# ikmb/vcf2prot

Measured on AMD Instinct MI355X. Metric: amino-acids written/sec, higher is better.
Workload: dtype u8

## Files before the change

### vcf2prot_amd/csrc/stitch_device.hpp

```cpp
#pragma once
#include <hip/hip_runtime.h>
#include <stdint.h>
#include "stitch_kernels.h"

namespace v2p {

typedef uint32_t u32x4 __attribute__((ext_vector_type(4)));
struct __attribute__((packed, aligned(1))) unaligned16 { u32x4 v; };

__device__ __forceinline__ u32x4 gather16(uint64_t addr)
{
    typedef const __attribute__((address_space(1))) unaligned16* gptr;
    return reinterpret_cast<gptr>(addr)->v;
}

struct __attribute__((packed, aligned(4))) dwaligned16 { u32x4 v; };
__device__ __forceinline__ u32x4 gather16_dw(uint64_t addr)
{
    typedef const __attribute__((address_space(1))) dwaligned16* gptr;
    typedef const __attribute__((address_space(1))) uint32_t* dptr;
    const uint64_t base = addr & ~3ull;
    const uint32_t sh = uint32_t(addr) & 3u;
    const u32x4 v = reinterpret_cast<gptr>(base)->v;
    const uint32_t e = *reinterpret_cast<dptr>(base + 16u);
// ... 100 lines not shown
            const uint32_t b0 = payload[src], b1 = payload[src + len - 1u];
            asm volatile("" :: "v"(b0), "v"(b1));
        }
    };
#pragma unroll
    for (uint32_t k = 0; k < TOUCH_CHUNKS_PER_WAVE; ++k) payload_lines(d[k]);
    for (uint32_t k = 0; k < TOUCH_CHUNKS_PER_WAVE; ++k) {
        const uint64_t n = (ch[k].dst_n >> 48) & uint64_t(CHUNK_N_MASK);
        const uint64_t tb = ch[k].task_begin & TB_IDX_MASK;
        for (uint64_t i = tb + 64u + lane; i < tb + n && i < n_desc; i += 64u) payload_lines(desc[i]);
    }
#pragma unroll
    for (uint32_t k = 0; k < TOUCH_CHUNKS_PER_WAVE; ++k) asm volatile("" :: "v"(d[k]));
}

}
```

### vcf2prot_amd/csrc/stitch_kernels.h

```cpp
#pragma once
#include <hip/hip_runtime.h>
#include <stdint.h>
#include "sir_pack.hpp"

namespace v2p {

enum : uint32_t {
    STATUS_BAD_CODE = 1,
    STATUS_RES_OOB = 2,
    STATUS_SRC_OOB = 3,
    STATUS_NOT_CONTIGUOUS = 4
};
constexpr unsigned long long STATUS_CLEAN = ~0ull;
constexpr int STITCH_TASKS_PER_LANE = 4;
constexpr uint32_t DOTS_BYTES = 64u * 1024u + 128u;

struct StitchArgs {
    const uint64_t* desc;
    uint64_t        n_desc;
    const Chunk*    chunks;
    uint32_t        n_chunks;
    const uint8_t*  src0;
    uint64_t        src0_len;
    const uint8_t*  src1;
// ... 4 lines not shown
    const uint8_t*  dots;
    const Chunk*    next_chunks = nullptr;
    uint32_t        n_next = 0;
    uint32_t        store_sc1 = 0;
    uint64_t        opt_phase_bytes = 0;
    uint32_t        opt_phase_min_chunks = 0;
    int32_t         opt_store_sc1 = -1;
    uint32_t        opt_touch = 0;
    uint32_t        rows = 0;
    uint64_t        img_desc = 0, img_bytes = 0;
    hipStream_t     aux_stream = nullptr;
    hipEvent_t      ev_fork = nullptr, ev_join = nullptr;
    uint32_t        opt_dual = 0;
    uint64_t*       stage = nullptr;
    uint32_t        stage_chunks = 0;
    const uint64_t* stage_cur = nullptr;
    uint64_t*       stage_next = nullptr;
    uint32_t        phase_chunks = 0;
};

uint32_t stitch_stage_chunks(const StitchArgs& args, int nontemporal);

struct OrderedArgs {
    const uint8_t*  code;
    const uint64_t* start_pos;
    const uint64_t* length;
    const uint64_t* start_pos_res;
    uint64_t        n_tasks;
    const uint8_t*  ref;
    const uint8_t*  alt;
    uint8_t*        res;
    uint64_t        esize;
};

struct ValidateArgs {
    const uint8_t*  code;
// ... 30 lines not shown
```

### vcf2prot_amd/csrc/stitch_kernels.hip

```cpp
#include <hip/hip_runtime.h>
#include <utility>
#include <vector>
#include <stdint.h>
#include <stdlib.h>
#include <mutex>
#include "stitch_kernels.h"
#include "stitch_device.hpp"

namespace v2p {

__device__ __forceinline__ u32x4 overwrite_tail(u32x4 v, u32x4 ld, uint32_t ja, bool take)
{
    const uint64_t x = ~0ull << (8u * (ja & 7u));
    const uint64_t mlo = (take && ja < 8u) ? x : 0ull;
    const uint64_t mhi = take ? (ja < 8u ? ~0ull : x) : 0ull;
    const uint32_t k0 = uint32_t(mlo), k1 = uint32_t(mlo >> 32), k2 = uint32_t(mhi), k3 = uint32_t(mhi >> 32);
    v[0] = (v[0] & ~k0) | (ld[0] & k0);
    v[1] = (v[1] & ~k1) | (ld[1] & k1);
    v[2] = (v[2] & ~k2) | (ld[2] & k2);
    v[3] = (v[3] & ~k3) | (ld[3] & k3);
    return v;
}

template <bool DW>
// ... 1009 lines not shown
    std::lock_guard<std::mutex> lk(mu);
    if (!bufs[dev]) {
        uint8_t* p = nullptr;
        *err = hipMalloc(reinterpret_cast<void**>(&p), DOTS_BYTES);
        if (*err != hipSuccess) return nullptr;
        *err = hipMemset(p, '.', DOTS_BYTES);
        if (*err == hipSuccess) *err = hipDeviceSynchronize();
        if (*err != hipSuccess) { (void)hipFree(p); return nullptr; }
        bufs[dev] = p;
    }
    return bufs[dev];
}


__global__ __launch_bounds__(256) void touch_image_kernel(const uint64_t* __restrict__ desc, const Chunk* __restrict__ chunks, uint32_t n_chunks, uint64_t n_desc,
                                                          const uint8_t* __restrict__ payload, uint64_t payload_len, uint64_t* __restrict__ stage)
{
    touch_chunks(desc, chunks, touch_wave_first(blockIdx.x & 7u, (blockIdx.x >> 3) * 4u + (threadIdx.x >> 6)), n_chunks, n_desc, payload, payload_len, threadIdx.x & 63u, stage);
}

static hipError_t launch_stitch_range(const StitchArgs& args, hipStream_t stream, int nontemporal, uint32_t max_blocks);

#ifdef V2P_BENCH_VARIANTS
__global__ void idle_kernel(uint32_t us)
{
    const uint64_t t0 = __builtin_readcyclecounter();
    while (__builtin_readcyclecounter() - t0 < uint64_t(us) * 100u) __builtin_amdgcn_s_sleep(64);
}
#endif

static uint64_t phase_plan(const StitchArgs& a, int nontemporal, uint32_t max_blocks, bool staged, bool* ride_out)
{
    *ride_out = false;
// ... 13 lines not shown
    per = per < per_min ? per_min : (per & ~7ull);
    const bool no_touch = (a.opt_touch & 1u) != 0, own_touch = (a.opt_touch & 2u) != 0;
    *ride_out = !own_touch && !no_touch && (nontemporal & 4) != 0 && (nontemporal & 48) == 48 && !(nontemporal & 2);
    return per;
}

uint32_t stitch_stage_chunks(const StitchArgs& args, int nontemporal)
{
    bool ride = false;
    const uint64_t per = phase_plan(args, nontemporal, 0, true, &ride);
    const int wsel = (nontemporal >> 28) & 3;
    if (!ride || !(nontemporal & 8) || wsel != 0 || (args.opt_touch & 4u) != 0 || args.opt_dual || per == 0 || per > 0x7FFFFFFFull) return 0;
    return uint32_t(per < args.n_chunks ? per : ((uint64_t(args.n_chunks) + 7u) & ~7ull));
}

hipError_t launch_stitch(const StitchArgs& args, hipStream_t stream, int nontemporal, uint32_t max_blocks)
{
    if (args.n_chunks == 0) return hipSuccess;
    StitchArgs a = args;
    hipError_t err = hipSuccess;
    a.dots = device_dots(&err);
    if (!a.dots) return err;
    a.rows = (nontemporal & 8) != 0;
    const uint64_t img_desc = a.img_desc ? a.img_desc : a.n_desc, img_bytes = a.img_bytes ? a.img_bytes : a.out_len;
    const bool rich = image_is_rich(img_desc, img_bytes);
    a.store_sc1 = a.opt_store_sc1 >= 0 ? uint32_t(a.opt_store_sc1 != 0) : uint32_t(!rich);
    bool ride = false;
    const uint64_t per = phase_plan(a, nontemporal, max_blocks, args.stage != nullptr && a.rows, &ride);
    if (per == 0) return launch_stitch_range(a, stream, nontemporal, max_blocks);
    const bool no_touch = (a.opt_touch & 1u) != 0;
    const int wsel = (nontemporal >> 28) & 3;
    if (ride && wsel == 0 && (a.opt_touch & 4u) != 0 && per <= 0x7FFFFFFFull) {
        const uint32_t n0 = uint32_t(args.n_chunks < per ? args.n_chunks : per);
        hipLaunchKernelGGL(touch_image_kernel, dim3(8u * ((touch_waves_per_xcd(n0) + 3u) / 4u)), dim3(256), 0, stream, a.desc, a.chunks, n0, a.n_desc, a.src1, a.src1_len, nullptr);
        a.phase_chunks = uint32_t(per);
        return launch_stitch_range(a, stream, nontemporal, 0);
    }
    if (ride && wsel == 0 && a.opt_dual && a.aux_stream && a.ev_fork && a.ev_join && args.n_chunks >= 4u * per) {
        const uint64_t half = (per / 2u) & ~7ull;
        std::vector<std::pair<uint64_t, uint32_t>> pieces;
        for (uint64_t c0 = 0; c0 < args.n_chunks; ) {
            uint64_t nc = pieces.size() == 1u ? (half / 2u) & ~7ull : half;
            if (nc == 0u) nc = 8u;
            if (nc > args.n_chunks - c0) nc = args.n_chunks - c0;
            pieces.emplace_back(c0, uint32_t(nc));
            c0 += nc;
        }
        err = hipEventRecord(a.ev_fork, stream);
        if (err == hipSuccess) err = hipStreamWaitEvent(a.aux_stream, a.ev_fork, 0);
        if (err != hipSuccess) return err;
        for (size_t i = 0; i < pieces.size(); ++i) {
            hipStream_t s = (i & 1u) ? a.aux_stream : stream;
            a.chunks = args.chunks + pieces[i].first;
            a.n_chunks = pieces[i].second;
            a.next_chunks = nullptr; a.n_next = 0;
            if (i + 2u < pieces.size()) { a.next_chunks = args.chunks + pieces[i + 2u].first; a.n_next = pieces[i + 2u].second; }
            if (i < 2u) hipLaunchKernelGGL(touch_image_kernel, dim3(8u * ((touch_waves_per_xcd(a.n_chunks) + 3u) / 4u)), dim3(256), 0, s, a.desc, a.chunks, a.n_chunks, a.n_desc, a.src1, a.src1_len, nullptr);
            err = launch_stitch_range(a, s, nontemporal, 0);
            if (err != hipSuccess) return err;
        }
        err = hipEventRecord(a.ev_join, a.aux_stream);
        if (err == hipSuccess) err = hipStreamWaitEvent(stream, a.ev_join, 0);
        return err != hipSuccess ? err : hipGetLastError();
    }
    const bool staged = ride && a.rows && wsel == 0 && args.stage != nullptr && per <= args.stage_chunks;
    uint32_t phase = 0;
    for (uint64_t c0 = 0; c0 < args.n_chunks; c0 += per, ++phase) {
        const uint32_t nc = uint32_t(args.n_chunks - c0 < per ? args.n_chunks - c0 : per);
        a.chunks = args.chunks + c0;
        a.n_chunks = nc;
        a.next_chunks = nullptr; a.n_next = 0;
        if (ride && c0 + per < args.n_chunks) {
            a.next_chunks = args.chunks + c0 + per;
            a.n_next = uint32_t(args.n_chunks - (c0 + per) < per ? args.n_chunks - (c0 + per) : per);
        }
        a.stage_cur = nullptr; a.stage_next = nullptr;
        if (staged) {
            a.stage_cur = args.stage + uint64_t(phase & 1u) * args.stage_chunks * STAGE_SLOTS;
            a.stage_next = args.stage + uint64_t((phase + 1u) & 1u) * args.stage_chunks * STAGE_SLOTS;
        }
        if (!no_touch && (!ride || c0 == 0)) hipLaunchKernelGGL(touch_image_kernel, dim3(8u * ((touch_waves_per_xcd(nc) + 3u) / 4u)), dim3(256), 0, stream, a.desc, a.chunks, nc, a.n_desc, a.src1, a.src1_len,
                                                                 staged ? const_cast<uint64_t*>(a.stage_cur) : nullptr);
        err = launch_stitch_range(a, stream, nontemporal, 0);
        if (err != hipSuccess) return err;
#ifdef V2P_BENCH_VARIANTS
        if (const char* e = getenv("V2P_PHASE_GAP_US")) hipLaunchKernelGGL(idle_kernel, dim3(1), dim3(64), 0, stream, uint32_t(atoi(e)));
        if (getenv("V2P_PHASE_SYNC")) (void)hipStreamSynchronize(stream);
#endif
    }
    return hipGetLastError();
}

static hipError_t launch_stitch_range(const StitchArgs& a, hipStream_t stream, int nontemporal, uint32_t max_blocks)
{
    hipError_t err = hipSuccess;
    const int nt = nontemporal & 1;
    const int var = (nontemporal >> 12) & 0xF;
// ... 124 lines not shown
```

### vcf2prot_amd/csrc/stitch_wave.hip

```cpp
#include <hip/hip_runtime.h>
#include <stdint.h>
#include <stdlib.h>
#include "stitch_kernels.h"
#include "stitch_device.hpp"

namespace v2p {

struct __attribute__((aligned(16))) WRec {
    uint32_t a_lo, a_hi;
    uint32_t se;
    uint32_t lit;
};
constexpr uint32_t WREC_NOLIT = 0xFFFFu;

__device__ __forceinline__ uint64_t wrec_adj(const WRec& t) { return (uint64_t(t.a_hi) << 32) | t.a_lo; }

__device__ __forceinline__ u32x4 put_byte(u32x4 v, uint32_t q, uint32_t byte)
{
    const uint32_t sh = 8u * (q & 3u), m = 0xFFu << sh, bv = byte << sh, k = q >> 2;
    v[0] = k == 0u ? (v[0] & ~m) | bv : v[0];
    v[1] = k == 1u ? (v[1] & ~m) | bv : v[1];
    v[2] = k == 2u ? (v[2] & ~m) | bv : v[2];
    v[3] = k == 3u ? (v[3] & ~m) | bv : v[3];
    return v;
// ... 33 lines not shown
    v[2] = (ld[2] & m[2]) | (v[2] & ~m[2]);
    v[3] = (ld[3] & m[3]) | (v[3] & ~m[3]);
    return v;
}

#ifndef V2P_WAVE_OCC
#define V2P_WAVE_OCC 8
#endif
template <int WPG, bool NT, bool SC1 = false, bool RIMG = false, bool STG = false>
__global__ __launch_bounds__(64 * WPG, V2P_WAVE_OCC) void stitchw_kernel(const uint64_t* __restrict__ p_desc, const Chunk* __restrict__ p_chunks,
                                                            const uint8_t* __restrict__ p_src0, const uint8_t* __restrict__ p_src1,
                                                            uint8_t* __restrict__ p_out, unsigned long long* __restrict__ p_status,
                                                            const uint8_t* __restrict__ p_dots,
                                                            uint32_t n_chunks, uint64_t n_desc, uint64_t src0_len, uint64_t src1_len, uint64_t out_len,
                                                            const Chunk* __restrict__ p_next, uint32_t n_next, uint32_t phase_chunks,
                                                            const uint64_t* __restrict__ p_stage = nullptr, uint64_t* __restrict__ p_stage_next = nullptr)
{
    static_assert(!STG || (RIMG && WPG == 1), "staged descriptors: rows images, one wave per workgroup");
    constexpr uint32_t ROWS = CHUNK_BYTES_WAVE / 1024u;
    static_assert(ROWS <= 16u, "a lane's map bytes and record indices are packed four rows to a register");
    constexpr uint32_t ND = (ROWS + 3u) / 4u;
    struct WaveLds {
        uint32_t map32[64u * ND];
        WRec rec[CHUNK_TASKS_WAVE + 4];
        u32x4 patch[CHUNK_TASKS_WAVE + 1];
    };
    __shared__ __attribute__((aligned(16))) WaveLds s_all[WPG];
    __shared__ u32x4 s_mask[17];
    __shared__ u32x4 s_one[17];

    const uint32_t lane = threadIdx.x & 63u;
// ... 1 lines not shown
    uint32_t c = blockIdx.x * uint32_t(WPG) + wid;
    if (WPG == 1 && phase_chunks != 0u) {
        const uint32_t tw = 8u * touch_waves_per_xcd(phase_chunks), per = tw + phase_chunks;
        const uint32_t g = blockIdx.x / per, r = blockIdx.x - g * per;
        if (r < tw) {
            const uint64_t base = uint64_t(g + 1u) * phase_chunks;
            if (base < n_chunks)
                touch_chunks(p_desc, p_chunks + base, touch_wave_first(r & 7u, r >> 3), uint32_t(n_chunks - base < phase_chunks ? n_chunks - base : phase_chunks),
                             n_desc, p_src1, src1_len, lane);
            return;
        }
        c = g * phase_chunks + (r - tw);
        if (c >= n_chunks) return;
    } else if (c >= n_chunks) {
        const uint32_t first_wg = (((n_chunks + uint32_t(WPG) - 1u) / uint32_t(WPG)) + 7u) & ~7u;
        if (blockIdx.x >= first_wg)
            touch_chunks(p_desc, p_next, touch_wave_first(blockIdx.x & 7u, ((blockIdx.x - first_wg) >> 3) * uint32_t(WPG) + wid), n_next, n_desc, p_src1, src1_len, lane,
                         STG ? p_stage_next : nullptr);
        return;
    }
    WaveLds& L = s_all[wid];
    uint64_t d_stg = 0ull;
    if (STG) d_stg = p_stage[uint64_t(c) * STAGE_SLOTS + lane];
    const uint64_t tb_raw = p_chunks[c].task_begin, dn = p_chunks[c].dst_n;
    if (!(dn & CHUNK_WAVE)) return;
    const uint64_t tb = RIMG ? tb_raw & TB_IDX_MASK : tb_raw;
    const uint32_t hskip = RIMG ? uint32_t(tb_raw >> TB_IDX_BITS) & PIECE_MAX : 0u;
    const uint32_t tclip = RIMG ? uint32_t(tb_raw >> (TB_IDX_BITS + TB_SKIP_BITS)) : 0u;
    const uint32_t n_hdr = uint32_t(dn >> 48) & CHUNK_N_MASK;
    if (RIMG != ((dn & CHUNK_CLIP) != 0ull)) { if (lane == 0u) report(p_status, tb, STATUS_RES_OOB); return; }
    const uint32_t n1 = RIMG ? uint32_t(dn & CHUNK_N1_MASK) : 0u;
    const uint64_t dst = RIMG ? dn & (DST_MASK & ~CHUNK_N1_MASK) : dn & DST_MASK;
    const uint32_t head = RIMG ? 0u : uint32_t(dst) & 15u;
// ... 217 lines not shown
    if (const char* e = getenv("V2P_WAVE_SUB")) sub = uint32_t(strtoul(e, nullptr, 10));
#endif
    if (sub == 0 || sub > a.n_chunks) sub = a.n_chunks;
    sub = (sub + 7u) & ~7u;
    for (uint32_t c0 = 0; c0 < a.n_chunks; c0 += sub) {
        const uint32_t nc = a.n_chunks - c0 < sub ? a.n_chunks - c0 : sub;
        const Chunk* ch = a.chunks + c0;
        const bool last = c0 + sub >= a.n_chunks;
        const uint32_t n_next = last && a.next_chunks ? a.n_next : 0u;
        const uint32_t tw = n_next ? touch_waves_per_xcd(n_next) : 0u;
#define V2P_LW(WW, NTT) hipLaunchKernelGGL((stitchw_kernel<WW, NTT>), dim3(tw ? ((((nc + (WW) - 1u) / (WW)) + 7u) & ~7u) + 8u * ((tw + (WW) - 1u) / (WW)) : (nc + (WW) - 1u) / (WW)), dim3(64 * (WW)), 0, stream, \
        a.desc, ch, a.src0, a.src1, a.out, a.status, a.dots, nc, a.n_desc, a.src0_len, a.src1_len, a.out_len, a.next_chunks, n_next, 0u)
#define V2P_LWR(NTT, SCC) hipLaunchKernelGGL((stitchw_kernel<1, NTT, SCC, true>), dim3(tw ? (((nc + 7u) & ~7u) + 8u * tw) : nc), dim3(64), 0, stream, \
        a.desc, ch, a.src0, a.src1, a.out, a.status, a.dots, nc, a.n_desc, a.src0_len, a.src1_len, a.out_len, a.next_chunks, n_next, 0u, nullptr, nullptr)
#define V2P_LWS(NTT, SCC) hipLaunchKernelGGL((stitchw_kernel<1, NTT, SCC, true, true>), dim3(tw ? (((nc + 7u) & ~7u) + 8u * tw) : nc), dim3(64), 0, stream, \
        a.desc, ch, a.src0, a.src1, a.out, a.status, a.dots, nc, a.n_desc, a.src0_len, a.src1_len, a.out_len, a.next_chunks, n_next, 0u, a.stage_cur, a.stage_next)
        if (a.rows && a.stage_cur && c0 == 0u && nc == a.n_chunks) {
            if (nt && a.store_sc1) V2P_LWS(true, true); else if (nt) V2P_LWS(true, false); else V2P_LWS(false, false);
        } else if (a.rows) { if (nt && a.store_sc1) V2P_LWR(true, true); else if (nt) V2P_LWR(true, false); else V2P_LWR(false, false); }
#ifdef V2P_BENCH_VARIANTS
        else if (waves_per_group == 4) { if (nt) V2P_LW(4, true); else V2P_LW(4, false); }
        else if (waves_per_group == 2) { if (nt) V2P_LW(2, true); else V2P_LW(2, false); }
#endif
        else if (nt && a.store_sc1) hipLaunchKernelGGL((stitchw_kernel<1, true, true>), dim3(tw ? (((nc + 7u) & ~7u) + 8u * tw) : nc), dim3(64), 0, stream,
                                                      a.desc, ch, a.src0, a.src1, a.out, a.status, a.dots, nc, a.n_desc, a.src0_len, a.src1_len, a.out_len, a.next_chunks, n_next, 0u);
        else { if (nt) V2P_LW(1, true); else V2P_LW(1, false); }
#undef V2P_LW
#undef V2P_LWR
#undef V2P_LWS
    }
    return hipGetLastError();
// ... 11 lines not shown
```

### vcf2prot_amd/csrc/v2p_api.hip

```cpp
#include <hip/hip_runtime.h>
#include <cstdint>
#include <cstdio>
#include <cstring>
#include <atomic>
#include <chrono>
#include <condition_variable>
#include <cstdlib>
#include <functional>
#include <memory>
#include <mutex>
#include <new>
#include <string>
#include <thread>
#include <vector>

#include "../../include/vcf2prot_hip.h"
#include "sir_pack.hpp"
#include "stitch_kernels.h"
#include "build_kernels.h"
#include "build_rows.h"
#include "dense_pieces.h"
#ifdef V2P_BENCH_VARIANTS
#include "patch_image.h"
#include "bench/v2p_bench.h"
// ... 139 lines not shown
    uint32_t tile_slots = 0;
    uint64_t tiles_n = 0;
    const uint32_t* tiles_count = nullptr;
    const uint64_t* tiles_res_base = nullptr;
    const uint8_t* payload_dev = nullptr;
    struct v2p_stream* from_stream = nullptr;
    bool orphaned = false;
    uint64_t pieces_src0_len = 0, pieces_src1_len = 0;
    DevBuf d_tiles, d_cover, d_pad, d_order;
    DevBuf d_pieces, d_chunks2;
    bool executed = false;
    uint64_t n_pieces = 0;
    int pieces_state = 0;
    PinnedBuf h_sum;
    DevBuf d_stage;
    bool pad_image = false;
    bool desc_swapped = false;
    uint64_t desc_slots = 0, pad_n_tiles = 0;
    uint32_t pad_K = 0;
    const uint64_t* pad_tdbase = nullptr;
    uint32_t n_slices = 0;
    uint64_t slice_chunk0[V2P_MAX_SLICES + 1] = {};
    uint64_t slice_desc[V2P_MAX_SLICES] = {}, slice_bytes[V2P_MAX_SLICES] = {};
    hipEvent_t ev_os[2 + 2 * V2P_MAX_SLICES] = {};
    hipEvent_t ev_aux[2] = {};
    hipEvent_t ev_par[V2P_MAX_SLICES] = {};
    bool os_ahead = false;
    float os_build_ms = 0.f;
    double os_wall_ms = 0.0;
    int os_kernel = 0;
// ... 1306 lines not shown
    } else if (n_chunks) HIP_TRY(c, hipMemcpyAsync(b->d_chunks.ptr(), a.chunks_tmp, n_chunks * sizeof(Chunk), hipMemcpyDeviceToDevice, c->stream), "D2D(chunks)");
    HIP_TRY(c, hipEventRecord(guard.ev[7], c->stream), "hipEventRecord");
    b->img.hap_out_begin.assign(n_h + 1, 0);
    HIP_TRY(c, hipMemcpyAsync(b->img.hap_out_begin.data(), b->d_hap.ptr(), (n_h + 1) * 8, hipMemcpyDeviceToHost, c->stream), "D2H(hap_begin)");
    rc = collect_status(c, b->d_status);
    if (rc) { (void)hipMemsetAsync(b->d_status.ptr(), 0xFF, 8, c->stream); return rc; }
    float ms0 = 0.f, ms1 = 0.f, ms2 = 0.f;
    (void)hipEventElapsedTime(&ms0, guard.ev[0], guard.ev[1]);
    (void)hipEventElapsedTime(&ms1, guard.ev[4], guard.ev[5]);
    (void)hipEventElapsedTime(&ms2, guard.ev[6], guard.ev[7]);
    if (build_ms) *build_ms = ms0 + ms_parse + ms1 + ms2;
    guard.ok = true;
    b->n_desc = n_desc; b->n_chunks = n_chunks; b->n_payload = v.n_alt; b->payload_dev = v.alt; b->out_bytes = out_bytes; b->n_haps = n_h;
    b->launch_hint = (mode == ROWS_DENSE ? 2 : 4) | 8 | 16 | 32 | (1 << 6) | (1 << 8);
    b->uses_proteome = true;
    b->finalized = true;
    b->n_slices = 0;
    return V2P_OK;
}

struct CheckErr { std::string msg; int64_t index = -1; int operator()(int code, const std::string& m, int64_t i = -1) { msg = m; index = i; return code; } };
static int check_stream_nolock(const v2p_ctx* c, const v2p_txstream* s, bool* fasta_out, std::vector<uint32_t>* arena_len, std::vector<uint64_t>* hap_out_begin, CheckErr& fail)
{
    if (!s->hap_tx_begin || (s->n_tx && (!s->tx_proteome_off || !s->tx_ref_len || !s->tx_res_len || !s->tx_task_begin || !s->tx_alt_begin)) ||
        (s->n_tasks && (!s->code || !s->start_pos || !s->length || !s->start_pos_res)) || (s->n_alt && !s->alt))
        return fail(V2P_ERR_INVALID_ARG, "null argument");
    if (s->hap_tx_begin[s->n_haps] != s->n_tx || (s->n_tx && (s->tx_task_begin[s->n_tx] != s->n_tasks || s->tx_alt_begin[s->n_tx] != s->n_alt)))
        return fail(V2P_ERR_INVALID_ARG, "stream offsets do not add up");
    if (s->hap_tx_begin[0] != 0) return fail(V2P_ERR_INVALID_ARG, "hap_tx_begin does not start at 0", 0);
    for (uint64_t h = 0; h < s->n_haps; ++h)
        if (s->hap_tx_begin[h + 1] < s->hap_tx_begin[h] || s->hap_tx_begin[h + 1] > s->n_tx)
// ... 207 lines not shown
    b->img.hap_out_begin.assign(n_h + 1, 0);
    HIP_TRY(c, hipMemcpyAsync(b->img.hap_out_begin.data(), b->d_hap.ptr(), (n_h + 1) * 8, hipMemcpyDeviceToHost, c->stream), "D2H(hap_begin)");
    rc = collect_status(c, b->d_status);
    float ms = 0.f, ms2 = 0.f;
    (void)hipEventElapsedTime(&ms, e0, e1);
    (void)hipEventElapsedTime(&ms2, e2, e3);
    ms += ms2;
    if (rc) { (void)hipMemsetAsync(b->d_status.ptr(), 0xFF, 8, c->stream); return rc; }
    guard.ok = true;
    if (build_ms) *build_ms = ms;
    b->n_desc = n_desc; b->n_chunks = n_chunks; b->n_payload = s->n_alt; b->payload_dev = b->d_payload.ptr(); b->out_bytes = out_bytes; b->n_haps = n_h;
    b->n_slices = 0;
    const int tpt = meta[3] <= 256u ? 1 : (meta[3] <= 512u ? 2 : 4);
    b->launch_hint = ((meta[0] & 2u) ? 2 : 0) | ((meta[0] & 4u) ? 4 : 0) | ((meta[0] & 1u) ? 0 : 16) | (meta[2] ? 0 : 32) | ((meta[1] ? 2 : 1) << 6) | (tpt << 8);
    b->uses_proteome = true;
    b->finalized = true;
    return V2P_OK;
#endif
}

#ifdef V2P_BENCH_VARIANTS
static int build_patch_image(v2p_batch* b, const DevStreamView& v, float* build_ms, bool own_stream_copy, uint64_t known_out_bytes)
{
    v2p_ctx* c = b->ctx;
    const uint64_t n_tx = v.n_tx, n_h = v.n_haps;
    struct Cleanup {
        hipEvent_t ev[2] = {nullptr, nullptr};
        DevBuf scratch;
        v2p_batch* b;
        bool ok = false, own;
        Cleanup(v2p_batch* b_, bool own_) : b(b_), own(own_) {}
// ... 75 lines not shown
    HIP_TRY(c, hipStreamSynchronize(c->stream), "hipStreamSynchronize");
    if (st != STATUS_CLEAN) {
        (void)hipMemsetAsync(b->d_status.ptr(), 0xFF, 8, c->stream);
        if (uint32_t(st & 0xFFu) == STATUS_PATCH_DECLINED) return c->fail(V2P_ERR_UNSUPPORTED, "a 8 KiB window of the result holds more segments or patches than a patch image's chunk (kernel 7 builds a dense image)", int64_t(st >> 8));
        const int code = reason_to_err(uint32_t(st & 0xFFu));
        return c->fail(code, std::string("device: ") + err_name(code) + " at descriptor " + std::to_string(st >> 8), int64_t(st >> 8));
    }
    float ms = 0.f;
    (void)hipEventElapsedTime(&ms, guard.ev[0], guard.ev[1]);
    if (build_ms) *build_ms = ms;
    guard.ok = true;
    b->n_desc = totals[0]; b->patch_segs = totals[0]; b->patch_patches = totals[1];
    b->n_chunks = n_chunks; b->n_payload = v.n_alt; b->payload_dev = v.alt; b->out_bytes = out_bytes; b->n_haps = n_h;
    b->launch_hint = 0; b->is_patch = true;
    b->uses_proteome = true;
    b->finalized = true;
    b->n_slices = 0;
    return V2P_OK;
}
#endif

struct v2p_stream {
    v2p_ctx* ctx = nullptr;
    DevBuf buf, alt;
    DevStreamView v;
    uint64_t out_bytes = 0;
    std::vector<uint64_t> hap_out_begin;
    DevBuf tiles;
    uint32_t tile_K = 0;
    uint64_t n_tiles = 0;
    const uint64_t* tile_res_base = nullptr;
// ... 126 lines not shown
    if (bpt >= double(WAVE_BYTES_PER_TASK)) return ROWS_WAVE;
    return ctx_variant(st->ctx) != 28u && tiles_possible(st) ? ROWS_TILES : ROWS_DENSE;
}

static int batch_reset_locked(v2p_batch* b, bool wait)
{
    v2p_ctx* c = b->ctx;
    HIP_TRY(c, hipSetDevice(c->device), "hipSetDevice");
    if (wait) HIP_TRY(c, hipStreamSynchronize(c->stream), "hipStreamSynchronize");
    b->img = ImageBuilder();
    b->finalized = false; b->uses_proteome = false; b->hap_open = false;
    b->n_desc = b->n_chunks = b->n_payload = b->out_bytes = b->n_haps = 0;
    b->payload_dev = nullptr; b->n_slices = 0; b->launch_hint = 0; b->is_patch = false; b->patch_segs = b->patch_patches = 0;
    b->is_tiles = false; b->tile_slots = 0; b->tiles_n = 0; b->tiles_count = nullptr; b->tiles_res_base = nullptr;
    b->pad_image = false; b->desc_slots = 0; b->pad_tdbase = nullptr; b->pieces_state = 0; b->executed = false;
    b->z_ready = false; b->z_begin.clear();
    b->os_kernel = 0; b->os_build_ms = 0.f; b->os_wall_ms = 0.0; b->os_ahead = false;
    stream_detach(b); b->orphaned = false;
    if (b->desc_swapped) { std::swap(b->d_desc, b->d_pad); b->desc_swapped = false; }
    return V2P_OK;
}

int v2p_batch_reset(v2p_batch* b)
{
    if (!b) return V2P_ERR_INVALID_ARG;
    std::lock_guard<std::mutex> lk(b->ctx->mu);
    const int rc = batch_reset_locked(b, true);
    b->d_z.release(); b->d_zws.release(); b->d_zbegin.release();
    return rc;
}
// ... 44 lines not shown

static void dual_of(v2p_ctx* c, StitchArgs& a)
{
    if (ctx_variant(c) != 19u) return;
    if (!c->exec_aux && hipStreamCreateWithFlags(&c->exec_aux, hipStreamNonBlocking) != hipSuccess) { c->exec_aux = nullptr; return; }
    for (hipEvent_t& e : c->ev_exec) if (!e && hipEventCreateWithFlags(&e, hipEventDisableTiming) != hipSuccess) { e = nullptr; return; }
    a.aux_stream = c->exec_aux; a.ev_fork = c->ev_exec[0]; a.ev_join = c->ev_exec[1]; a.opt_dual = 1u;
}

static hipError_t ensure_event(hipEvent_t& e) { return e ? hipSuccess : hipEventCreate(&e); }

static hipError_t attach_stage(v2p_batch* b, StitchArgs& a, int hint)
{
    const uint64_t idesc = a.img_desc ? a.img_desc : a.n_desc, ibytes = a.img_bytes ? a.img_bytes : a.out_len;
    const bool small_rich = image_is_rich(idesc, ibytes) && a.src0_len <= PHASE_STAGED_SMALL_REF && 8u * idesc + 16u * uint64_t(a.n_chunks) >= 8u * PHASE_BYTES_RICH;
    if (ctx_variant(b->ctx) == 23u || !(b->pad_image || ctx_variant(b->ctx) == 25u || small_rich)) return hipSuccess;
    const uint32_t rows = stitch_stage_chunks(a, hint);
    if (rows == 0) return hipSuccess;
    const hipError_t e = b->d_stage.ensure(uint64_t(2) * rows * 64u * 8u);
    if (e != hipSuccess) { (void)hipGetLastError(); return hipSuccess; }
    a.stage = reinterpret_cast<uint64_t*>(b->d_stage.ptr()); a.stage_chunks = rows;
    return hipSuccess;
}

static hipError_t stitch_range(v2p_batch* b, uint64_t desc_bound, uint64_t chunk0, uint64_t n_chunks, uint64_t img_desc, uint64_t img_bytes, hipStream_t stream)
{
    v2p_ctx* c = b->ctx;
    if (n_chunks == 0) return hipSuccess;
    StitchArgs a{reinterpret_cast<const uint64_t*>(b->d_desc.ptr()), desc_bound, reinterpret_cast<const Chunk*>(b->d_chunks.ptr()) + chunk0,
                 uint32_t(n_chunks), c->proteome.ptr(), c->proteome_len + c->headers_len, b->payload_dev, b->n_payload,
                 b->d_out.ptr(), b->out_bytes, reinterpret_cast<unsigned long long*>(b->d_status.ptr())};
    a.opt_phase_bytes = c->launch_opts.phase_bytes; a.opt_phase_min_chunks = c->launch_opts.phase_min_chunks; a.opt_store_sc1 = c->launch_opts.store_sc1;
    a.opt_touch = touch_of(ctx_variant(c));
// ... 195 lines not shown
    }
    if (ahead) {
        OS_TRY(hipStreamWaitEvent(A, b->ev_os[3 + 2 * (S - 1)], 0), "hipStreamWaitEvent");
        b->slice_chunk0[S] = chunk0;
        for (uint32_t j = 0; j < S; ++j)
            OS_TRY(stitch_range(b, desc_cap, b->slice_chunk0[j], b->slice_chunk0[j + 1] - b->slice_chunk0[j], b->slice_desc[j], b->slice_bytes[j], A), "launch(stitch)");
    }
#undef OS_TRY
#undef OS_ALLOC
#undef ensure_exact
    b->slice_chunk0[S] = chunk0;
    HIP_TRY(c, hipEventRecord(b->ev_os[1], A), "hipEventRecord");
    b->n_desc = desc0; b->n_chunks = chunk0; b->n_slices = S;
    b->img.hap_out_begin = st->hap_out_begin;
    b->uses_proteome = true;
    b->finalized = true;
    return V2P_OK;
}

static hipError_t tiles_execute(v2p_batch* b, hipStream_t stream)
{
    v2p_ctx* c = b->ctx;
    TileExecArgs a{reinterpret_cast<const uint64_t*>(b->d_desc.ptr()), b->tile_slots, b->tiles_count, b->tiles_res_base, b->tiles_n,
                   c->proteome.ptr(), b->payload_dev, b->d_out.ptr(), b->out_bytes, reinterpret_cast<const unsigned long long*>(b->d_status.ptr())};
    return launch_stitch_tiles(a, stream, !(c->flags & V2P_FLAG_TEMPORAL));
}

static int build_tiles(v2p_batch* b, const v2p_stream* st, bool execute, bool* fallback, float* build_ms, uint32_t n_slices)
{
    v2p_ctx* c = b->ctx;
    const DevStreamView& v = st->v;
// ... 83 lines not shown
    const unsigned long long stw = hs[6];
    if (stw != STATUS_CLEAN) {
        (void)hipMemsetAsync(b->d_status.ptr(), 0xFF, 8, A);
        const uint32_t reason = uint32_t(stw & 0xFFu);
        if (reason == STATUS_ROWS_STAGE || reason == STATUS_ROWS_TOO_MANY) { *fallback = true; return V2P_OK; }
        if (reason == STATUS_ROWS_SPAN) return c->fail(V2P_ERR_UNSUPPORTED, "64 consecutive transcripts with more than 2 GiB of result", int64_t(stw >> 8));
        const int code = reason_to_err(reason);
        return c->fail(code, std::string("device: ") + err_name(code) + " at descriptor " + std::to_string(stw >> 8), int64_t(stw >> 8));
    }
    if (hs[5] != out_bytes) return c->fail(V2P_ERR_STATE, "the resident stream's tables changed since its upload");
    b->is_tiles = true; b->tile_slots = slots; b->tiles_n = n_tiles; b->tiles_count = a.tile_count; b->tiles_res_base = a.tile_res_base;
    b->n_desc = hs[4]; b->n_chunks = n_tiles; b->n_payload = v.n_alt; b->payload_dev = v.alt; b->out_bytes = out_bytes; b->n_haps = n_h;
    b->pieces_src0_len = c->proteome_len + c->headers_len; b->pieces_src1_len = v.n_alt;
    b->launch_hint = 0; b->pad_image = false; b->desc_slots = 0;
    b->img.hap_out_begin = st->hap_out_begin;
    b->uses_proteome = true; b->finalized = true;
    b->n_slices = 1; b->slice_chunk0[0] = 0; b->slice_chunk0[1] = n_tiles; b->os_ahead = false;
    if (execute && !executed_in_slices) HIP_TRY(c, tiles_execute(b, A), "launch(stitch: tile image)");
    HIP_TRY(c, hipEventRecord(b->ev_os[1], A), "hipEventRecord");
    if (build_ms) { *build_ms = 0.f; (void)hipEventElapsedTime(build_ms, b->ev_os[0], b->ev_os[3]); }
    return V2P_OK;
}

static int build_and_execute_locked(v2p_batch* b, const v2p_stream* st, int kernel, uint32_t n_slices)
{
    v2p_ctx* c = b->ctx;
    if (b->finalized) return c->fail(V2P_ERR_STATE, "batch already finalized (v2p_batch_reset recycles it)");
    if (b->hap_open || b->img.n_haplotypes()) return c->fail(V2P_ERR_STATE, "the batch already holds host-built haplotypes");
    if (kernel != 0 && kernel != 6 && kernel != 7 && kernel != 8 && kernel != 9) return c->fail(V2P_ERR_INVALID_ARG, "a resident stream builds rows images (kernel 6, 7), a patch image (8), a tile image (9) or what the routing rule picks (0)");
    HIP_TRY(c, hipSetDevice(c->device), "hipSetDevice");
    const auto t0 = std::chrono::steady_clock::now();
// ... 111 lines not shown
        const hipError_t me = b->d_pad.ensure((b->n_desc ? b->n_desc : 1) * 8);
        if (me == hipErrorOutOfMemory) { (void)hipGetLastError(); return V2P_OK; }
        HIP_TRY(c, me, "hipMalloc(dense descriptors)");
    }
    if (b->n_desc) {
        RowsArgs a{};
        a.n_tiles = b->pad_n_tiles; a.K = b->pad_K; a.tile0 = 0; a.tile1 = b->pad_n_tiles;
        a.tile_desc_base = const_cast<uint64_t*>(b->pad_tdbase);
        a.desc_pad = reinterpret_cast<uint64_t*>(b->d_desc.ptr()); a.desc = reinterpret_cast<uint64_t*>(b->d_pad.ptr()); a.desc_cap = b->n_desc;
        HIP_TRY(c, launch_rows_compact(a, c->stream), "launch(compact)");
    }
    if (b->n_chunks) HIP_TRY(c, launch_rows_chunks_dense(reinterpret_cast<const Chunk*>(b->d_chunks.ptr()), b->n_chunks, b->pad_tdbase, reinterpret_cast<Chunk*>(b->d_chunks.ptr()), c->stream), "launch(chunk records)");
    std::swap(b->d_desc, b->d_pad);
    b->desc_swapped = !b->desc_swapped;
    b->pad_image = false; b->desc_slots = 0;
    return V2P_OK;
}

int v2p_batch_download_image(v2p_batch* b, uint64_t* desc, v2p_chunk* chunks, uint64_t* hap_out_begin)
{
    if (!b) return V2P_ERR_INVALID_ARG;
    v2p_ctx* c = b->ctx;
    std::lock_guard<std::mutex> lk(c->mu);
    if (!b->finalized) return c->fail(V2P_ERR_STATE, "batch not finalized");
    if (b->is_patch && desc) return c->fail(V2P_ERR_STATE, "a patch image has segments and patches, not descriptors: v2p_batch_download_patch_image");
    if (b->is_tiles && (desc || chunks)) return c->fail(V2P_ERR_STATE, "a tile image has pieces in its tiles' slots, not descriptors and chunks (v2p_batch_build_from_stream with kernel 7 builds the dense rows image of the same stream)");
    HIP_TRY(c, hipSetDevice(c->device), "hipSetDevice");
    if (b->pad_image) { const int rc = densify(b); if (rc) return rc; }
    if (b->pad_image) return c->fail(V2P_ERR_HIP, "no device memory for the dense copy of a padded image");
    if (desc && b->n_desc) HIP_TRY(c, hipMemcpyAsync(desc, b->d_desc.ptr(), b->n_desc * 8, hipMemcpyDeviceToHost, c->stream), "D2H(desc)");
// ... 49 lines not shown
    HIP_TRY(c, b->d_payload.ensure(b->n_payload), "hipMalloc(payload)");
    HIP_TRY(c, b->d_out.ensure((b->out_bytes + 15) & ~15ull), "hipMalloc(out)");
    HIP_TRY(c, b->d_hap.ensure((b->n_haps + 1) * 8), "hipMalloc(hap_begin)");
    HIP_TRY(c, b->d_digest.ensure((b->n_haps ? b->n_haps : 1) * 8), "hipMalloc(digest)");
    if (b->n_desc) HIP_TRY(c, hipMemcpyAsync(b->d_desc.ptr(), b->img.desc.data(), b->n_desc * 8, hipMemcpyHostToDevice, c->stream), "H2D(desc)");
    if (b->n_chunks) HIP_TRY(c, hipMemcpyAsync(b->d_chunks.ptr(), b->img.chunks.data(), b->n_chunks * sizeof(Chunk), hipMemcpyHostToDevice, c->stream), "H2D(chunks)");
    if (b->n_payload) HIP_TRY(c, hipMemcpyAsync(b->d_payload.ptr(), b->img.payload.data(), b->n_payload, hipMemcpyHostToDevice, c->stream), "H2D(payload)");
    HIP_TRY(c, hipMemcpyAsync(b->d_hap.ptr(), b->img.hap_out_begin.data(), (b->n_haps + 1) * 8, hipMemcpyHostToDevice, c->stream), "H2D(hap_begin)");
    b->payload_dev = b->d_payload.ptr();
    int rc = init_status(c, b->d_status);
    if (rc) return rc;
    HIP_TRY(c, hipStreamSynchronize(c->stream), "hipStreamSynchronize");
    std::vector<uint64_t>().swap(b->img.desc);
    std::vector<Chunk>().swap(b->img.chunks);
    std::vector<uint8_t>().swap(b->img.payload);
    b->finalized = true;
    return V2P_OK;
}

static bool pieces_eligible(const v2p_batch* b)
{
    const int h = b->launch_hint;
    return b->finalized && !b->is_patch && !b->is_tiles && (h & 2) && (h & 8) && !(h & 4) && (h & 16) && (h & 32) && b->n_chunks != 0 && ctx_variant(b->ctx) != 28u &&
           ctx_variant(b->ctx) != 3u && ctx_variant(b->ctx) != 8u;
}
static int to_pieces(v2p_batch* b)
{
    v2p_ctx* c = b->ctx;
    if (b->pieces_state != 0) return V2P_OK;
    b->pieces_state = -1;
    DevBuf cnt, basebuf, scratch, st;
// ... 89 lines not shown
    if (!b) return V2P_ERR_INVALID_ARG;
    std::lock_guard<std::mutex> lk(b->ctx->mu);
    const bool f = b->finalized;
    if (n_haps) *n_haps = f ? b->n_haps : b->img.n_haplotypes();
    if (n_desc) *n_desc = f ? b->n_desc : b->img.desc.size();
    if (n_chunks) *n_chunks = f ? b->n_chunks : b->img.chunks.size();
    if (out_bytes) *out_bytes = f ? b->out_bytes : b->img.out_size();
    if (payload_bytes) *payload_bytes = f ? b->n_payload : b->img.payload.size();
    return V2P_OK;
}

int v2p_batch_image_form(const v2p_batch* b)
{
    if (!b) return V2P_ERR_INVALID_ARG;
    std::lock_guard<std::mutex> lk(b->ctx->mu);
    return (b->pad_image ? 1 : 0) | (b->pieces_state == 1 ? 2 : 0) | (b->d_stage.ptr() ? 4 : 0) | (b->is_tiles ? 8 : 0);
}

int v2p_batch_hap_range(const v2p_batch* b, uint64_t h, uint64_t* begin, uint64_t* len)
{
    if (!b || !begin || !len) return V2P_ERR_INVALID_ARG;
    std::lock_guard<std::mutex> lk(b->ctx->mu);
    const std::vector<uint64_t>& hb = b->img.hap_out_begin;
    if (h + 1 >= hb.size()) return V2P_ERR_INVALID_ARG;
    *begin = hb[h]; *len = hb[h + 1] - hb[h];
    return V2P_OK;
}

int v2p_batch_download(v2p_batch* b, uint64_t begin, uint64_t len, uint8_t* out)
{
    if (!b || (len && !out)) return V2P_ERR_INVALID_ARG;
// ... 668 lines not shown
```

### vcf2prot_amd/engine.py

```python
from __future__ import annotations

import ctypes
import enum
import os
from dataclasses import dataclass
from typing import Dict, List, Optional, Sequence, Tuple

import numpy as np

from . import _native as N
from ._native import V2PError


class Engine(enum.Enum):
    ST = 0
    MT = 1
    GPU = 2

    @staticmethod
    def from_str(name: str) -> "Engine":
        out = ctypes.c_int(-1)
        rc = N.hip_lib().v2p_engine_from_str(name.encode(), ctypes.byref(out))
        if rc != N.V2P_OK:
            raise ValueError(f"{name} is not a supported engine")
# ... 305 lines not shown

    def build_from_stream(self, rs: "ResidentStream", kernel: int = 0) -> float:
        ms = ctypes.c_float(0.0)
        self.ctx._check(self._lib.v2p_batch_build_from_stream(self._h, rs._h, kernel, ctypes.byref(ms)))
        self._stream_ref = rs
        return float(ms.value)

    def build_and_execute(self, rs: "ResidentStream", kernel: int = 0, n_slices: int = 0):
        self.ctx._check(self._lib.v2p_batch_build_and_execute(self._h, rs._h, kernel, n_slices))
        self._stream_ref = rs

    def image_form(self) -> dict:
        f = self._lib.v2p_batch_image_form(self._h)
        if f < 0:
            self.ctx._check(f)
        return {"padded": bool(f & 1), "pieces": bool(f & 2), "staging_buffers": bool(f & 4), "tiles": bool(f & 8)}

    def oneshot_info(self) -> dict:
        info = N.OneShotInfo()
        self.ctx._check(self._lib.v2p_batch_oneshot_info(self._h, ctypes.byref(info)))
        return {"kernel": int(info.kernel), "n_slices": int(info.n_slices), "total_ms": float(info.total_ms), "build_ms": float(info.build_ms),
                "call_wall_ms": float(info.call_wall_ms), "tables_ms": float(info.tables_ms), "slice_build_ms": [float(info.slice_build_ms[j]) for j in range(int(info.n_slices))]}

    def reset(self):
        self.ctx._check(self._lib.v2p_batch_reset(self._h))

    def download_patch_image(self):
        n = self.counts()["n_chunks"]
        seg = np.zeros((n, 1024), dtype=np.uint64)
        patch = np.zeros((n, 1024), dtype=np.uint32)
        chunks = np.zeros((n, 2), dtype=np.uint64)
# ... 176 lines not shown
```

Before: 4964 billion.

## Keep a resident per-chunk descriptor slot image across repeated batch executions

After a batch has executed once, a full-size slot buffer is allocated that holds every chunk's 64 descriptor slots, and it is filled once by the touch kernel. Later executions read descriptors from this resident buffer instead of re-gathering them into double-buffered staging each phase. The touch pass then only reads the slots and prefetches payload lines, through a new `touch_slots` path. The cost is extra device memory proportional to the chunk count, plus invalidation bookkeeping whenever the image changes; a missed invalidation would leave stale descriptors in use.

```diff
diff --git a/vcf2prot_amd/csrc/stitch_device.hpp b/vcf2prot_amd/csrc/stitch_device.hpp
--- a/vcf2prot_amd/csrc/stitch_device.hpp
+++ b/vcf2prot_amd/csrc/stitch_device.hpp
@@ -138,4 +138,28 @@
     for (uint32_t k = 0; k < TOUCH_CHUNKS_PER_WAVE; ++k) asm volatile("" :: "v"(d[k]));
 }
 
+__device__ __forceinline__ void touch_slots(const uint64_t* __restrict__ slots, const Chunk* __restrict__ chunks, uint32_t c0, uint32_t n_chunks,
+                                            const uint8_t* __restrict__ payload, uint64_t payload_len, uint32_t lane)
+{
+    if (c0 >= n_chunks) return;
+    Chunk ch[TOUCH_CHUNKS_PER_WAVE];
+    uint64_t d[TOUCH_CHUNKS_PER_WAVE];
+#pragma unroll
+    for (uint32_t k = 0; k < TOUCH_CHUNKS_PER_WAVE; ++k) {
+        const uint32_t c = c0 + 8u * k < n_chunks ? c0 + 8u * k : c0;
+        ch[k] = chunks[c];
+        d[k] = slots[uint64_t(c) * STAGE_SLOTS + lane];
+    }
+#pragma unroll
+    for (uint32_t k = 0; k < TOUCH_CHUNKS_PER_WAVE; ++k) {
+        const uint64_t src = d[k] & SRC_MASK, len = (d[k] >> 40) & LEN_MASK;
+        if ((d[k] >> 62) == SPACE_PAYLOAD && len != 0u && src < payload_len && len <= payload_len - src) {
+            const uint32_t b0 = payload[src], b1 = payload[src + len - 1u];
+            asm volatile("" :: "v"(b0), "v"(b1));
+        }
+    }
+#pragma unroll
+    for (uint32_t k = 0; k < TOUCH_CHUNKS_PER_WAVE; ++k) asm volatile("" :: "v"(d[k]), "v"(ch[k].task_begin), "v"(ch[k].dst_n));
 }
+
+}
diff --git a/vcf2prot_amd/csrc/stitch_kernels.h b/vcf2prot_amd/csrc/stitch_kernels.h
--- a/vcf2prot_amd/csrc/stitch_kernels.h
+++ b/vcf2prot_amd/csrc/stitch_kernels.h
@@ -42,12 +42,14 @@
     uint32_t        opt_dual = 0;
     uint64_t*       stage = nullptr;
     uint32_t        stage_chunks = 0;
+    uint32_t        stage_resident = 0;
     const uint64_t* stage_cur = nullptr;
     uint64_t*       stage_next = nullptr;
     uint32_t        phase_chunks = 0;
 };
 
 uint32_t stitch_stage_chunks(const StitchArgs& args, int nontemporal);
+hipError_t launch_stage_slots(const StitchArgs& args, uint64_t* slots, hipStream_t stream);
 
 struct OrderedArgs {
     const uint8_t*  code;
diff --git a/vcf2prot_amd/csrc/stitch_kernels.hip b/vcf2prot_amd/csrc/stitch_kernels.hip
--- a/vcf2prot_amd/csrc/stitch_kernels.hip
+++ b/vcf2prot_amd/csrc/stitch_kernels.hip
@@ -1047,9 +1047,11 @@
 
 
 __global__ __launch_bounds__(256) void touch_image_kernel(const uint64_t* __restrict__ desc, const Chunk* __restrict__ chunks, uint32_t n_chunks, uint64_t n_desc,
-                                                          const uint8_t* __restrict__ payload, uint64_t payload_len, uint64_t* __restrict__ stage)
-{
-    touch_chunks(desc, chunks, touch_wave_first(blockIdx.x & 7u, (blockIdx.x >> 3) * 4u + (threadIdx.x >> 6)), n_chunks, n_desc, payload, payload_len, threadIdx.x & 63u, stage);
+                                                          const uint8_t* __restrict__ payload, uint64_t payload_len, uint64_t* __restrict__ stage, uint32_t resident)
+{
+    const uint32_t c0 = touch_wave_first(blockIdx.x & 7u, (blockIdx.x >> 3) * 4u + (threadIdx.x >> 6));
+    if (resident) touch_slots(stage, chunks, c0, n_chunks, payload, payload_len, threadIdx.x & 63u);
+    else touch_chunks(desc, chunks, c0, n_chunks, n_desc, payload, payload_len, threadIdx.x & 63u, stage);
 }
 
 static hipError_t launch_stitch_range(const StitchArgs& args, hipStream_t stream, int nontemporal, uint32_t max_blocks);
@@ -1093,6 +1095,14 @@
     return uint32_t(per < args.n_chunks ? per : ((uint64_t(args.n_chunks) + 7u) & ~7ull));
 }
 
+hipError_t launch_stage_slots(const StitchArgs& args, uint64_t* slots, hipStream_t stream)
+{
+    if (args.n_chunks == 0) return hipSuccess;
+    hipLaunchKernelGGL(touch_image_kernel, dim3(8u * ((touch_waves_per_xcd(args.n_chunks) + 3u) / 4u)), dim3(256), 0, stream, args.desc, args.chunks, args.n_chunks, args.n_desc,
+                       args.src1, args.src1_len, slots, 0u);
+    return hipGetLastError();
+}
+
 hipError_t launch_stitch(const StitchArgs& args, hipStream_t stream, int nontemporal, uint32_t max_blocks)
 {
     if (args.n_chunks == 0) return hipSuccess;
@@ -1111,7 +1121,7 @@
     const int wsel = (nontemporal >> 28) & 3;
     if (ride && wsel == 0 && (a.opt_touch & 4u) != 0 && per <= 0x7FFFFFFFull) {
         const uint32_t n0 = uint32_t(args.n_chunks < per ? args.n_chunks : per);
-        hipLaunchKernelGGL(touch_image_kernel, dim3(8u * ((touch_waves_per_xcd(n0) + 3u) / 4u)), dim3(256), 0, stream, a.desc, a.chunks, n0, a.n_desc, a.src1, a.src1_len, nullptr);
+        hipLaunchKernelGGL(touch_image_kernel, dim3(8u * ((touch_waves_per_xcd(n0) + 3u) / 4u)), dim3(256), 0, stream, a.desc, a.chunks, n0, a.n_desc, a.src1, a.src1_len, nullptr, 0u);
         a.phase_chunks = uint32_t(per);
         return launch_stitch_range(a, stream, nontemporal, 0);
     }
@@ -1134,7 +1144,7 @@
             a.n_chunks = pieces[i].second;
             a.next_chunks = nullptr; a.n_next = 0;
             if (i + 2u < pieces.size()) { a.next_chunks = args.chunks + pieces[i + 2u].first; a.n_next = pieces[i + 2u].second; }
-            if (i < 2u) hipLaunchKernelGGL(touch_image_kernel, dim3(8u * ((touch_waves_per_xcd(a.n_chunks) + 3u) / 4u)), dim3(256), 0, s, a.desc, a.chunks, a.n_chunks, a.n_desc, a.src1, a.src1_len, nullptr);
+            if (i < 2u) hipLaunchKernelGGL(touch_image_kernel, dim3(8u * ((touch_waves_per_xcd(a.n_chunks) + 3u) / 4u)), dim3(256), 0, s, a.desc, a.chunks, a.n_chunks, a.n_desc, a.src1, a.src1_len, nullptr, 0u);
             err = launch_stitch_range(a, s, nontemporal, 0);
             if (err != hipSuccess) return err;
         }
@@ -1142,7 +1152,9 @@
         if (err == hipSuccess) err = hipStreamWaitEvent(stream, a.ev_join, 0);
         return err != hipSuccess ? err : hipGetLastError();
     }
-    const bool staged = ride && a.rows && wsel == 0 && args.stage != nullptr && per <= args.stage_chunks;
+    const bool resident = args.stage_resident != 0 && args.n_chunks <= args.stage_chunks;
+    const bool staged = ride && a.rows && wsel == 0 && args.stage != nullptr && (resident || (args.stage_resident == 0 && per <= args.stage_chunks));
+    a.stage_resident = staged && resident;
     uint32_t phase = 0;
     for (uint64_t c0 = 0; c0 < args.n_chunks; c0 += per, ++phase) {
         const uint32_t nc = uint32_t(args.n_chunks - c0 < per ? args.n_chunks - c0 : per);
@@ -1154,12 +1166,15 @@
             a.n_next = uint32_t(args.n_chunks - (c0 + per) < per ? args.n_chunks - (c0 + per) : per);
         }
         a.stage_cur = nullptr; a.stage_next = nullptr;
-        if (staged) {
+        if (staged && resident) {
+            a.stage_cur = args.stage + c0 * STAGE_SLOTS;
+            a.stage_next = args.stage + (c0 + nc) * STAGE_SLOTS;
+        } else if (staged) {
             a.stage_cur = args.stage + uint64_t(phase & 1u) * args.stage_chunks * STAGE_SLOTS;
             a.stage_next = args.stage + uint64_t((phase + 1u) & 1u) * args.stage_chunks * STAGE_SLOTS;
         }
         if (!no_touch && (!ride || c0 == 0)) hipLaunchKernelGGL(touch_image_kernel, dim3(8u * ((touch_waves_per_xcd(nc) + 3u) / 4u)), dim3(256), 0, stream, a.desc, a.chunks, nc, a.n_desc, a.src1, a.src1_len,
-                                                                 staged ? const_cast<uint64_t*>(a.stage_cur) : nullptr);
+                                                                 staged ? const_cast<uint64_t*>(a.stage_cur) : nullptr, a.stage_resident);
         err = launch_stitch_range(a, stream, nontemporal, 0);
         if (err != hipSuccess) return err;
 #ifdef V2P_BENCH_VARIANTS
diff --git a/vcf2prot_amd/csrc/stitch_wave.hip b/vcf2prot_amd/csrc/stitch_wave.hip
--- a/vcf2prot_amd/csrc/stitch_wave.hip
+++ b/vcf2prot_amd/csrc/stitch_wave.hip
@@ -71,7 +71,7 @@
                                                             const uint8_t* __restrict__ p_dots,
                                                             uint32_t n_chunks, uint64_t n_desc, uint64_t src0_len, uint64_t src1_len, uint64_t out_len,
                                                             const Chunk* __restrict__ p_next, uint32_t n_next, uint32_t phase_chunks,
-                                                            const uint64_t* __restrict__ p_stage = nullptr, uint64_t* __restrict__ p_stage_next = nullptr)
+                                                            const uint64_t* __restrict__ p_stage = nullptr, uint64_t* __restrict__ p_stage_next = nullptr, uint32_t stage_resident = 0u)
 {
     static_assert(!STG || (RIMG && WPG == 1), "staged descriptors: rows images, one wave per workgroup");
     constexpr uint32_t ROWS = CHUNK_BYTES_WAVE / 1024u;
@@ -103,9 +103,11 @@
         if (c >= n_chunks) return;
     } else if (c >= n_chunks) {
         const uint32_t first_wg = (((n_chunks + uint32_t(WPG) - 1u) / uint32_t(WPG)) + 7u) & ~7u;
-        if (blockIdx.x >= first_wg)
-            touch_chunks(p_desc, p_next, touch_wave_first(blockIdx.x & 7u, ((blockIdx.x - first_wg) >> 3) * uint32_t(WPG) + wid), n_next, n_desc, p_src1, src1_len, lane,
-                         STG ? p_stage_next : nullptr);
+        if (blockIdx.x >= first_wg) {
+            const uint32_t t0 = touch_wave_first(blockIdx.x & 7u, ((blockIdx.x - first_wg) >> 3) * uint32_t(WPG) + wid);
+            if (STG && stage_resident) touch_slots(p_stage_next, p_next, t0, n_next, p_src1, src1_len, lane);
+            else touch_chunks(p_desc, p_next, t0, n_next, n_desc, p_src1, src1_len, lane, STG ? p_stage_next : nullptr);
+        }
         return;
     }
     WaveLds& L = s_all[wid];
@@ -353,7 +355,7 @@
 #define V2P_LWR(NTT, SCC) hipLaunchKernelGGL((stitchw_kernel<1, NTT, SCC, true>), dim3(tw ? (((nc + 7u) & ~7u) + 8u * tw) : nc), dim3(64), 0, stream, \
         a.desc, ch, a.src0, a.src1, a.out, a.status, a.dots, nc, a.n_desc, a.src0_len, a.src1_len, a.out_len, a.next_chunks, n_next, 0u, nullptr, nullptr)
 #define V2P_LWS(NTT, SCC) hipLaunchKernelGGL((stitchw_kernel<1, NTT, SCC, true, true>), dim3(tw ? (((nc + 7u) & ~7u) + 8u * tw) : nc), dim3(64), 0, stream, \
-        a.desc, ch, a.src0, a.src1, a.out, a.status, a.dots, nc, a.n_desc, a.src0_len, a.src1_len, a.out_len, a.next_chunks, n_next, 0u, a.stage_cur, a.stage_next)
+        a.desc, ch, a.src0, a.src1, a.out, a.status, a.dots, nc, a.n_desc, a.src0_len, a.src1_len, a.out_len, a.next_chunks, n_next, 0u, a.stage_cur, a.stage_next, a.stage_resident)
         if (a.rows && a.stage_cur && c0 == 0u && nc == a.n_chunks) {
             if (nt && a.store_sc1) V2P_LWS(true, true); else if (nt) V2P_LWS(true, false); else V2P_LWS(false, false);
         } else if (a.rows) { if (nt && a.store_sc1) V2P_LWR(true, true); else if (nt) V2P_LWR(true, false); else V2P_LWR(false, false); }
diff --git a/vcf2prot_amd/csrc/v2p_api.hip b/vcf2prot_amd/csrc/v2p_api.hip
--- a/vcf2prot_amd/csrc/v2p_api.hip
+++ b/vcf2prot_amd/csrc/v2p_api.hip
@@ -177,6 +177,8 @@
     int pieces_state = 0;
     PinnedBuf h_sum;
     DevBuf d_stage;
+    uint64_t slots_chunks = 0;
+    bool slots_no_room = false;
     bool pad_image = false;
     bool desc_swapped = false;
     uint64_t desc_slots = 0, pad_n_tiles = 0;
@@ -1513,7 +1515,7 @@
     b->n_desc = n_desc; b->n_chunks = n_chunks; b->n_payload = v.n_alt; b->payload_dev = v.alt; b->out_bytes = out_bytes; b->n_haps = n_h;
     b->launch_hint = (mode == ROWS_DENSE ? 2 : 4) | 8 | 16 | 32 | (1 << 6) | (1 << 8);
     b->uses_proteome = true;
-    b->finalized = true;
+    b->finalized = true; b->slots_chunks = 0;
     b->n_slices = 0;
     return V2P_OK;
 }
@@ -1751,7 +1753,7 @@
     const int tpt = meta[3] <= 256u ? 1 : (meta[3] <= 512u ? 2 : 4);
     b->launch_hint = ((meta[0] & 2u) ? 2 : 0) | ((meta[0] & 4u) ? 4 : 0) | ((meta[0] & 1u) ? 0 : 16) | (meta[2] ? 0 : 32) | ((meta[1] ? 2 : 1) << 6) | (tpt << 8);
     b->uses_proteome = true;
-    b->finalized = true;
+    b->finalized = true; b->slots_chunks = 0;
     return V2P_OK;
 #endif
 }
@@ -1857,7 +1859,7 @@
     b->n_chunks = n_chunks; b->n_payload = v.n_alt; b->payload_dev = v.alt; b->out_bytes = out_bytes; b->n_haps = n_h;
     b->launch_hint = 0; b->is_patch = true;
     b->uses_proteome = true;
-    b->finalized = true;
+    b->finalized = true; b->slots_chunks = 0;
     b->n_slices = 0;
     return V2P_OK;
 }
@@ -2014,6 +2016,7 @@
     b->payload_dev = nullptr; b->n_slices = 0; b->launch_hint = 0; b->is_patch = false; b->patch_segs = b->patch_patches = 0;
     b->is_tiles = false; b->tile_slots = 0; b->tiles_n = 0; b->tiles_count = nullptr; b->tiles_res_base = nullptr;
     b->pad_image = false; b->desc_slots = 0; b->pad_tdbase = nullptr; b->pieces_state = 0; b->executed = false;
+    b->slots_chunks = 0; b->slots_no_room = false;
     b->z_ready = false; b->z_begin.clear();
     b->os_kernel = 0; b->os_build_ms = 0.f; b->os_wall_ms = 0.0; b->os_ahead = false;
     stream_detach(b); b->orphaned = false;
@@ -2088,9 +2091,24 @@
 {
     const uint64_t idesc = a.img_desc ? a.img_desc : a.n_desc, ibytes = a.img_bytes ? a.img_bytes : a.out_len;
     const bool small_rich = image_is_rich(idesc, ibytes) && a.src0_len <= PHASE_STAGED_SMALL_REF && 8u * idesc + 16u * uint64_t(a.n_chunks) >= 8u * PHASE_BYTES_RICH;
-    if (ctx_variant(b->ctx) == 23u || !(b->pad_image || ctx_variant(b->ctx) == 25u || small_rich)) return hipSuccess;
+    const uint32_t var = ctx_variant(b->ctx);
+    if (var == 23u || !(b->pad_image || var == 25u || var == 30u || small_rich)) return hipSuccess;
     const uint32_t rows = stitch_stage_chunks(a, hint);
     if (rows == 0) return hipSuccess;
+    const bool whole = a.chunks == reinterpret_cast<const Chunk*>(b->d_chunks.ptr()) && a.n_chunks == b->n_chunks;
+    if (b->executed && !b->pad_image && whole && var != 26u && var != 30u && !b->slots_no_room) {
+        if (b->slots_chunks != b->n_chunks) {
+            b->slots_chunks = 0;
+            if (b->d_stage.ensure_exact(b->n_chunks * uint64_t(64u * 8u)) != hipSuccess) { (void)hipGetLastError(); b->slots_no_room = true; }
+            else if (launch_stage_slots(a, reinterpret_cast<uint64_t*>(b->d_stage.ptr()), b->ctx->stream) != hipSuccess) (void)hipGetLastError();
+            else b->slots_chunks = b->n_chunks;
+        }
+        if (b->slots_chunks == b->n_chunks) {
+            a.stage = reinterpret_cast<uint64_t*>(b->d_stage.ptr()); a.stage_chunks = uint32_t(b->n_chunks); a.stage_resident = 1u;
+            return hipSuccess;
+        }
+    }
+    b->slots_chunks = 0;
     const hipError_t e = b->d_stage.ensure(uint64_t(2) * rows * 64u * 8u);
     if (e != hipSuccess) { (void)hipGetLastError(); return hipSuccess; }
     a.stage = reinterpret_cast<uint64_t*>(b->d_stage.ptr()); a.stage_chunks = rows;
@@ -2316,7 +2334,7 @@
     b->n_desc = desc0; b->n_chunks = chunk0; b->n_slices = S;
     b->img.hap_out_begin = st->hap_out_begin;
     b->uses_proteome = true;
-    b->finalized = true;
+    b->finalized = true; b->slots_chunks = 0;
     return V2P_OK;
 }
 
@@ -2430,7 +2448,7 @@
     b->pieces_src0_len = c->proteome_len + c->headers_len; b->pieces_src1_len = v.n_alt;
     b->launch_hint = 0; b->pad_image = false; b->desc_slots = 0;
     b->img.hap_out_begin = st->hap_out_begin;
-    b->uses_proteome = true; b->finalized = true;
+    b->uses_proteome = true; b->finalized = true; b->slots_chunks = 0;
     b->n_slices = 1; b->slice_chunk0[0] = 0; b->slice_chunk0[1] = n_tiles; b->os_ahead = false;
     if (execute && !executed_in_slices) HIP_TRY(c, tiles_execute(b, A), "launch(stitch: tile image)");
     HIP_TRY(c, hipEventRecord(b->ev_os[1], A), "hipEventRecord");
@@ -2572,6 +2590,7 @@
     std::swap(b->d_desc, b->d_pad);
     b->desc_swapped = !b->desc_swapped;
     b->pad_image = false; b->desc_slots = 0;
+    b->slots_chunks = 0;
     return V2P_OK;
 }
 
@@ -2651,7 +2670,7 @@
     std::vector<uint64_t>().swap(b->img.desc);
     std::vector<Chunk>().swap(b->img.chunks);
     std::vector<uint8_t>().swap(b->img.payload);
-    b->finalized = true;
+    b->finalized = true; b->slots_chunks = 0;
     return V2P_OK;
 }
 
@@ -2771,7 +2790,7 @@
 {
     if (!b) return V2P_ERR_INVALID_ARG;
     std::lock_guard<std::mutex> lk(b->ctx->mu);
-    return (b->pad_image ? 1 : 0) | (b->pieces_state == 1 ? 2 : 0) | (b->d_stage.ptr() ? 4 : 0) | (b->is_tiles ? 8 : 0);
+    return (b->pad_image ? 1 : 0) | (b->pieces_state == 1 ? 2 : 0) | (b->d_stage.ptr() ? 4 : 0) | (b->is_tiles ? 8 : 0) | (b->slots_chunks ? 16 : 0);
 }
 
 int v2p_batch_hap_range(const v2p_batch* b, uint64_t h, uint64_t* begin, uint64_t* len)
diff --git a/vcf2prot_amd/engine.py b/vcf2prot_amd/engine.py
--- a/vcf2prot_amd/engine.py
+++ b/vcf2prot_amd/engine.py
@@ -343,7 +343,7 @@
         f = self._lib.v2p_batch_image_form(self._h)
         if f < 0:
             self.ctx._check(f)
-        return {"padded": bool(f & 1), "pieces": bool(f & 2), "staging_buffers": bool(f & 4), "tiles": bool(f & 8)}
+        return {"padded": bool(f & 1), "pieces": bool(f & 2), "staging_buffers": bool(f & 4), "tiles": bool(f & 8), "resident_slots": bool(f & 16)}
 
     def oneshot_info(self) -> dict:
         info = N.OneShotInfo()
```

Result: slower. 4772 billion (-3.9%).
